# barry-mir/mixing-style-transfer

Hardware: AMD Instinct MI355X
Metric: triplets/sec (10 s @ 44.1 kHz, 4-stem, bs=24) (higher is better)
Workload: dtype f32

## Files before the change

### mixing-style-transfer_amd/csrc/melfeat.hip

```cpp
#include "common.h"
#include "fft_wave.h"
#include "fft_pk.h"
#include "stage_a_tables.h"

#include <algorithm>
#include <cmath>
#include <memory>
#include <vector>


namespace {

constexpr int kWaves = 8;
constexpr int kFPW = 2;
constexpr int kTF = kWaves * kFPW;
constexpr int kTileStride = kTF + 1;
constexpr int kThreads = kWaves * 64;
constexpr int nf_of(int n_fft) { return n_fft >= 2048 ? 1 : kFPW; }
constexpr int kNumScalars = 80;

enum : int {
  S_LOGSUM = 0,
  S_LINSUM = 4,
  S_MASK = 8,
// ... 688 lines not shown
          p.logmel[((size_t)clip * 8 * M + row) * p.F + fb + f] = s_tile[f * TS + row];
    }
    for (int e = tid; e < nf * M; e += kThreads) {
      const int f = e / M, m = e - f * M;
      const float* t = s_tile + f * TS + m;
      float S[4];
#pragma unroll
      for (int s = 0; s < 4; ++s)
        S[s] = 0.5f * ((__expf(t[(2 * s) * M]) - 1e-10f) + (__expf(t[(2 * s + 1) * M]) - 1e-10f));
#pragma unroll
      for (int s = 0; s < 4; ++s) {
        float other = -INFINITY;
#pragma unroll
        for (int j = 0; j < 4; ++j)
          if (j != s) other = fmaxf(other, S[j]);
        mask[s] += __frcp_rn(1.0f + __expf(S[s] - other));
      }
    }
    {
      const int b0 = fb * p.hop, b1 = (fb + nf == p.F) ? p.T : min(p.T, (fb + nf) * p.hop);
      for (int i = b0 + tid * 4; i < b1; i += kThreads * 4) {
        float x[8][4];
#pragma unroll
        for (int c = 0; c < 8; ++c) {
          const ST* src = chan(c) + i;
          if (i + 3 < b1) {
            Smp<ST>::ld4(src, x[c]);
          } else {
#pragma unroll
            for (int e = 0; e < 4; ++e) x[c][e] = (i + e < b1) ? Smp<ST>::ld(src + e) : 0.f;
          }
        }
#pragma unroll
        for (int e = 0; e < 4; ++e) {
          const float mL = ((x[0][e] + x[2][e]) + x[4][e]) + x[6][e];
          const float mR = ((x[1][e] + x[3][e]) + x[5][e]) + x[7][e];
          mixsq = fmaf(mL, mL, mixsq);
          mixsq = fmaf(mR, mR, mixsq);
        }
      }
    }
    __syncthreads();
  }

  float* red = reinterpret_cast<float*>(s_scr);
#pragma unroll
  for (int r = 0; r < NB; ++r) red[(wave * NB + r) * 64 + lane] = acc_db[r];
  float* red2 = red + kWaves * NB * 64;
  {
    const float v[13] = {acc_log, acc_lin, sqL, sqR, dsL, dsR, dqL, dqR, cr, mid, side, mixsq, 0.f};
#pragma unroll
    for (int k = 0; k < 12; ++k) {
      const float r = mst::wave_sum(v[k]);
      if (lane == 0) red2[wave * 24 + k] = r;
    }
    const float a = mst::wave_max(pkL), b = mst::wave_max(pkR);
#pragma unroll
    for (int s = 0; s < 4; ++s) {
      const float r = mst::wave_sum(mask[s]);
      if (lane == 0) red2[wave * 24 + 14 + s] = r;
    }
    if (lane == 0) red2[wave * 24 + 12] = a, red2[wave * 24 + 13] = b;
  }
  __syncthreads();
  for (int i = tid; i < 4 * NB * 64; i += kThreads) {
    const int l = i & 63, r = (i >> 6) % NB, s = i / (64 * NB);
    const int band = p.lanebands[r * 64 + l].band;
    if (band >= 0) {
      float v = 0.f;
#pragma unroll
      for (int w = 0; w < WPS; ++w) v += red[((WPS * s + w) * NB + r) * 64 + l];
      part[s * M + band] = v;
    }
  }
  if (tid < 4) {
    const int s = tid;
    float v[14];
#pragma unroll
    for (int k = 0; k < 14; ++k) v[k] = 0.f;
    for (int w = 0; w < WPS; ++w) {
      const float* a = red2 + (WPS * s + w) * 24;
#pragma unroll
      for (int k = 0; k < 12; ++k) v[k] += a[k];
      v[12] = fmaxf(v[12], a[12]), v[13] = fmaxf(v[13], a[13]);
    }
    float* q = part + 4 * M;
    q[S_LOGSUM + s] = v[0];
    q[S_LINSUM + s] = v[1];
    q[S_SQ + 2 * s] = v[2], q[S_SQ + 2 * s + 1] = v[3];
    q[S_DSUM + 2 * s] = v[4], q[S_DSUM + 2 * s + 1] = v[5];
    q[S_DSQ + 2 * s] = v[6], q[S_DSQ + 2 * s + 1] = v[7];
    q[S_CROSS + s] = v[8];
    q[S_MID + s] = v[9];
    q[S_SIDE + s] = v[10];
    q[S_PEAK + 2 * s] = v[12], q[S_PEAK + 2 * s + 1] = v[13];
    float mk = 0.f;
    for (int w = 0; w < kWaves; ++w) mk += red2[w * 24 + 14 + s];
    q[S_MASK + s] = mk;
    q[S_PIVOT + 2 * s] = Smp<ST>::ld(chan(2 * s) + o_piv), q[S_PIVOT + 2 * s + 1] = Smp<ST>::ld(chan(2 * s + 1) + o_piv);
  }
  if (tid == 8) {
    float mx = 0.f;
    for (int w = 0; w < kWaves; ++w) mx += red2[w * 24 + 11];
    part[4 * M + S_MIX] = mx;
    part[4 * M + S_NSAMP] = (float)max(0, o_end - o_begin);
    part[4 * M + S_NFRAME] = (float)max(0, f_end - f_begin);
  }
}

struct FParams {
  const float* partials;
  float* feats;
  int M, F, T, runs_per_clip, pstride, detailed_bins, feat_dim;
};

__device__ __forceinline__ double wave_sum_f64(double v) {
#pragma unroll
  for (int o = 32; o > 0; o >>= 1) v += __shfl_xor(v, o, 64);
  return v;
}

__device__ double pearson_vs_index(const double* y, int n, int lane) {
  double my = 0;
  for (int i = lane; i < n; i += 64) my += y[i];
  my = wave_sum_f64(my) / n;
  const double mx = 0.5 * (n - 1);
  double sxy = 0, sxx = 0, syy = 0;
  for (int i = lane; i < n; i += 64) {
    const double dx = i - mx, dy = y[i] - my;
    sxy += dx * dy, sxx += dx * dx, syy += dy * dy;
  }
  sxy = wave_sum_f64(sxy), sxx = wave_sum_f64(sxx), syy = wave_sum_f64(syy);
  const double std_unbiased = sqrt(syy / (n - 1));
  if (std_unbiased < 1e-6) return 0.0;
  double c = sxy / sqrt(sxx * syy);
  return fmin(1.0, fmax(-1.0, c));
}

struct FinalizeLds {
  static constexpr int a_sc = 0, a_chmean = a_sc + kNumScalars * 8, a_chm2 = a_chmean + 64, a_cross = a_chm2 + 64, a_curve = a_cross + 64;
  static constexpr size_t bytes(int M, int detailed_bins) { return (size_t)4 * M * 8 + a_curve + (size_t)4 * (detailed_bins > 0 ? detailed_bins : 0) * 8; }
};

__global__ __launch_bounds__(256) void melfeat_finalize_kernel(const FParams p) {
  extern __shared__ __attribute__((aligned(16))) unsigned char smem[];
  using L = FinalizeLds;
  double* band = reinterpret_cast<double*>(smem);
  unsigned char* after_band = reinterpret_cast<unsigned char*>(band + 4 * p.M);
  double* sc = reinterpret_cast<double*>(after_band + L::a_sc);
  double* chmean = reinterpret_cast<double*>(after_band + L::a_chmean);
  double* chm2 = reinterpret_cast<double*>(after_band + L::a_chm2);
  double* cross = reinterpret_cast<double*>(after_band + L::a_cross);
  const int tid = threadIdx.x, clip = blockIdx.x, M = p.M;
  const float* base = p.partials + (size_t)clip * p.runs_per_clip * p.pstride;
  const double inv_n_db = 1.0 / (2.0 * p.F);
  const double k_db = 10.0 / log(10.0);
  for (int i = tid; i < 4 * M; i += 256) {
    double s = 0;
#pragma unroll 8
    for (int r = 0; r < p.runs_per_clip; ++r) s += base[(size_t)r * p.pstride + i];
    band[i] = s * inv_n_db * k_db;
  }
  if (tid < kNumScalars) {
    const bool is_max = tid >= S_PEAK && tid < S_PEAK + 8;
    double s = 0;
#pragma unroll 8
    for (int r = 0; r < p.runs_per_clip; ++r) {
      const double v = base[(size_t)r * p.pstride + 4 * M + tid];
      s = is_max ? fmax(s, v) : s + v;
    }
    sc[tid] = s;
  }
  if (tid < 8) {
    double n = 0, mean = 0, m2 = 0;
    for (int r = 0; r < p.runs_per_clip; ++r) {
      const float* q = base + (size_t)r * p.pstride + 4 * M;
      const double nr = q[S_NSAMP];
      if (nr <= 0) continue;
      const double sr = q[S_DSUM + tid], qr = q[S_DSQ + tid];
      const double mr = q[S_PIVOT + tid] + sr / nr, m2r = fmax(0.0, qr - sr * sr / nr);
      const double d = mr - mean, nt = n + nr;
      m2 += m2r + d * d * n * nr / nt;
      mean += d * nr / nt;
      n = nt;
    }
    chmean[tid] = mean, chm2[tid] = m2;
  } else if (tid >= 64 && tid < 68) {
    const int s = tid - 64;
    double n = 0, mL = 0, mR = 0, c = 0;
    for (int r = 0; r < p.runs_per_clip; ++r) {
      const float* q = base + (size_t)r * p.pstride + 4 * M;
      const double nr = q[S_NSAMP];
      if (nr <= 0) continue;
      const double sL = q[S_DSUM + 2 * s], sR = q[S_DSUM + 2 * s + 1];
      const double mLr = q[S_PIVOT + 2 * s] + sL / nr, mRr = q[S_PIVOT + 2 * s + 1] + sR / nr;
      const double cr = q[S_CROSS + s] - sL * sR / nr;
      const double dL = mLr - mL, dR = mRr - mR, nt = n + nr;
      c += cr + dL * dR * n * nr / nt;
      mL += dL * nr / nt, mR += dR * nr / nt;
      n = nt;
    }
    cross[s] = c;
  }
  __syncthreads();

  const int sd = p.detailed_bins > 0 ? p.detailed_bins + 2 : 5;
  const int ps = 10 + sd;
  float* out = p.feats + (size_t)clip * p.feat_dim;
  const int lane = tid & 63;
  auto put_lane = [&](int idx, double v) {
    float f = (float)v;
    f = fminf(fmaxf(f, -100.0f), 100.0f);
    if (v != v) f = 0.0f;
    out[idx] = f;
  };
  auto put = [&](int idx, double v) {
    if (lane == 0) put_lane(idx, v);
  };
  const double n = (double)p.T;
  auto loud = [&](double ms) { return -0.691 + 10.0 * log10(ms + 1e-10); };
  {
    const int s = tid >> 6;
    const int blk = (s == 1) ? 0 : (s == 2) ? ps : (s == 3) ? 2 * ps + 4 : 3 * ps + 4;
    const double msL = sc[S_SQ + 2 * s] / n, msR = sc[S_SQ + 2 * s + 1] / n;
    const double rmsL = sqrt(msL), rmsR = sqrt(msR);
    const double l_stem = loud((sc[S_SQ + 2 * s] + sc[S_SQ + 2 * s + 1]) / (2 * n));
    const double l_mix = loud(sc[S_MIX] / (2 * n));
    put(blk + 0, rmsL);
    put(blk + 1, rmsR);
    put(blk + 2, 20.0 * log10(sc[S_PEAK + 2 * s] / (rmsL + 1e-8)));
    put(blk + 3, 20.0 * log10(sc[S_PEAK + 2 * s + 1] / (rmsR + 1e-8)));
    put(blk + 4, l_stem);
    put(blk + 5, l_stem);
    put(blk + 6, l_stem - l_mix);
    const double* e = band + s * M;
    const double cnt = 2.0 * M * p.F;
    const double flat = exp(sc[S_LOGSUM + s] / cnt) / (sc[S_LINSUM + s] / cnt + 1e-10);
    int o = blk + 7;
    if (p.detailed_bins == 0) {
      const int q = M / 4;
      double lo = 0, mi = 0, hi = 0;
      for (int i = lane; i < q; i += 64) lo += e[i];
      for (int i = q + lane; i < 3 * q; i += 64) mi += e[i];
      for (int i = 3 * q + lane; i < M; i += 64) hi += e[i];
      lo = wave_sum_f64(lo), mi = wave_sum_f64(mi), hi = wave_sum_f64(hi);
      put(o + 0, lo / q);
      put(o + 1, mi / (2 * q));
      put(o + 2, hi / (M - 3 * q));
      put(o + 3, pearson_vs_index(e, M, lane));
      put(o + 4, flat);
    } else {
      const int nb = p.detailed_bins;
      double* curve = reinterpret_cast<double*>(after_band + L::a_curve) + s * nb;
      for (int i = lane; i < nb; i += 64) {
        if (nb >= M) { curve[i] = e[i]; continue; }
        const float scale = nb > 1 ? (float)(M - 1) / (float)(nb - 1) : 0.f;
        const float src = scale * i;
        int i0 = (int)src;
        if (i0 > M - 1) i0 = M - 1;
        const int i1 = i0 + (i0 < M - 1 ? 1 : 0);
        const double lam = src - (float)i0;
        curve[i] = (1.0 - lam) * e[i0] + lam * e[i1];
      }
      __syncthreads();
      for (int i = lane; i < nb; i += 64) put_lane(o + i, curve[i]);
      put(o + nb, pearson_vs_index(curve, nb, lane));
      put(o + nb + 1, flat);
    }
    o = blk + 7 + sd;
    put(o + 0, 20.0 * log10(rmsL / (rmsR + 1e-8)));
    put(o + 1, cross[s] / (sqrt(chm2[2 * s] * chm2[2 * s + 1]) + 1e-8));
    put(o + 2, (sc[S_SIDE + s] / (4 * n)) / (sc[S_MID + s] / (4 * n) + 1e-8));
    put(2 * ps + s, sc[S_MASK + s] / ((double)M * p.F));
  }
}

template <auto Kernel, typename Params>
int launch_stage_a(const Params& kp, int grid, int threads, size_t lds, hipStream_t st) {
  MST_REQUIRE(lds <= kMaxLds, "mst_melfeat_forward: LDS %zu B exceeds 160 KiB", lds);
  const hipError_t e = mst::launch_lds<Kernel>(dim3(grid), dim3(threads), lds, st, kp);
  if (e != hipSuccess) return mst::fail(MST_EHIP, "stage-A kernel launch failed: %s", hipGetErrorString(e));
  return MST_OK;
}

template <int NFFT, int NB, typename ST>
int launch_melfeat(const KParams& kp, int grid, hipStream_t st) {
  return launch_stage_a<melfeat_kernel<NFFT, NB, ST>>(kp, grid, kThreads, GenericLds<NFFT>::bytes(kp.tw_count, kp.tw2_count, kp.nnz, kp.M, kp.tile_bufs), st);
}
template <int NFFT, typename ST, int WPS>
int launch_melfeat_spw(const KParams& kp, int grid, hipStream_t st) {
  return launch_stage_a<melfeat_spw_kernel<NFFT, ST, WPS>>(kp, grid, SpwGeom<WPS>::THREADS, SpwLds<NFFT, WPS>::bytes(kp.tw2_count, kp.nnz, kp.M), st);
}

#include "melfeat_v2.inc"
#include "melfeat_v2_2048.inc"

}

static_assert(sizeof(stage_a::F2) == sizeof(float2), "stage_a_tables.h's pairs are uploaded as float2");

struct mst_plan {
  int sr, n_fft, hop, n_mels, detailed_bins, feat_dim;
  int batches_per_run;
  mst::DevBuf<float> window;
  struct {
    int nb, nnz, tw_count, tw2_count, glen[4], goff[4];
    mst::DevBuf<float2> tw, tw2, post;
    mst::DevBuf<float> melw;
    mst::DevBuf<LaneBand> lanebands;
  } gen;
  struct {
    bool ok = false;
    int wps = 3;
    int nslot = 0, maxcnt = 0, segw_count = 0, glen[kV2Slots] = {0}, goff[kV2Slots] = {0};
    mst::DevBuf<float2> tw2, tw3, tw4, segw;
    mst::DevBuf<int> start, id, bandtab;
  } sw;
};

namespace {

struct StageAEnv {
  int batches_per_run, spw_wps;
  bool v2_wps2, generic, v2_nostd;
  bool old_kernels;
};
StageAEnv read_stage_a_env() {
  auto num = [](const char* name, int dflt) { const char* e = getenv(name); return e ? atoi(e) : dflt; };
  const char* a = getenv("MST_STAGE_A");
  StageAEnv s;
  s.batches_per_run = getenv("MST_MELFEAT_BATCHES") ? std::max(1, num("MST_MELFEAT_BATCHES", 0)) : 0;
  s.spw_wps = num("MST_SPW_WPS", 3);
  s.v2_wps2 = num("MST_V2_WPS", 0) == 2, s.generic = getenv("MST_MELFEAT_GENERIC"), s.v2_nostd = getenv("MST_V2_NOSTD");
  s.old_kernels = s.generic || (a && (!strcmp(a, "spw") || !strcmp(a, "generic")));
  return s;
}

int frames_per_run_of(const mst_plan* p, int F) {
  if (p->batches_per_run > 0) return p->batches_per_run * kTF;
  int fpr = (F + 31) / 32;
  fpr += fpr & 1;
  return std::max(2 * kTF, fpr);
}
int runs_per_clip(const mst_plan* p, int F) {
  const int fpr = frames_per_run_of(p, F);
  return (F + fpr - 1) / fpr;
}
int pstride_of(const mst_plan* p) { return 4 * p->n_mels + kNumScalars; }

int sw_fpw(const mst_plan* p, int F) { return std::max(1, ((F + 31) / 32 + p->sw.wps - 1) / p->sw.wps); }
int sw_runs(const mst_plan* p, int F) {
  const int fpr = p->sw.wps * sw_fpw(p, F);
  return (F + fpr - 1) / fpr;
}

bool v2_table_is_standard(const mst_plan* p) {
  const auto& t = p->sw;
  return p->n_mels == 128 && t.nslot == 3 && t.maxcnt == 1 && t.glen[0] == 14 && t.glen[1] == 3 && !t.glen[2] && !t.goff[0] && t.goff[1] == 14 && t.goff[2] == 17;
}

}

extern "C" {

int mst_plan_create(mst_plan** out, int sample_rate, int n_fft, int hop, int n_mels, const float* window,
                    const float* fb, int detailed_bins) {
  MST_REQUIRE(out && window && fb, "mst_plan_create: NULL argument");
  *out = nullptr;
  MST_REQUIRE(n_fft == 512 || n_fft == 1024 || n_fft == 2048,
              "mst_plan_create: n_fft=%d unsupported (512, 1024, 2048)", n_fft);
  MST_REQUIRE(hop >= 1 && n_mels >= 4 && n_mels <= 256, "mst_plan_create: bad hop=%d / n_mels=%d", hop, n_mels);
  MST_REQUIRE(detailed_bins >= 0 && detailed_bins <= 256 && (detailed_bins == 0 || detailed_bins < n_mels ||
              detailed_bins == n_mels), "mst_plan_create: bad detailed_bins=%d", detailed_bins);
  std::unique_ptr<mst_plan> p(new mst_plan());
  p->sr = sample_rate, p->n_fft = n_fft, p->hop = hop, p->n_mels = n_mels, p->detailed_bins = detailed_bins;
  const int sd = detailed_bins > 0 ? detailed_bins + 2 : 5;
  p->feat_dim = 4 * (10 + sd) + 4;
  const StageAEnv env = read_stage_a_env();
  p->batches_per_run = env.batches_per_run;
  const int n_bins = n_fft / 2 + 1;
  auto& g = p->gen;
  auto& sw = p->sw;
  const bool v2 = n_fft == 1024 && hop == 256, v4 = n_fft == 2048 && hop == 512 && n_mels <= 128;
  sw.wps = (env.v2_wps2 || n_mels > 128 || v4) ? 2 : 3;
  stage_a::PieceTable t;
  if (v2 || v4) t = stage_a::build_pieces(fb, n_bins, n_mels, v2 ? stage_a::v2_piece_opts(n_mels) : stage_a::v4_piece_opts());
  sw.ok = t.ok, sw.nslot = t.nslot, sw.maxcnt = t.maxcnt, sw.segw_count = (int)t.segw.size();
  for (int r = 0; r < kV2Slots; ++r) sw.glen[r] = t.glen[r], sw.goff[r] = t.goff[r];
  const std::vector<int> bands = !t.ok ? std::vector<int>() : v2 ? stage_a::pack_bands16(t, n_mels, stage_a::kV2Dump) : stage_a::pack_bands8(t, n_mels);
  std::vector<float2> t2(mstpk::kTw2Rows * 64), t3(mstpk::kTw3Rows * 64);
  mstpk::fill_twiddles_host(t2.data(), t3.data());
  const std::vector<stage_a::F2> t4 = v4 ? stage_a::tw4_twiddles() : std::vector<stage_a::F2>();

  g.nb = n_mels <= 128 ? 2 : 4;
  const stage_a::LaneBandTable lb = stage_a::build_lane_bands(fb, n_bins, n_mels, g.nb);
  g.nnz = lb.nnz;
  for (int r = 0; r < 4; ++r) g.glen[r] = lb.glen[r], g.goff[r] = lb.goff[r];
  const std::vector<stage_a::F2> tw = stage_a::fft_twiddles(n_fft / 2), post = stage_a::post_twiddles(n_fft);
  std::vector<stage_a::F2> tw2;
  if (n_fft <= 1024) tw2 = stage_a::fft_twiddles(n_fft);
  g.tw_count = (int)tw.size(), g.tw2_count = (int)tw2.size();
  if (tw2.empty()) tw2.push_back(stage_a::F2{1.f, 0.f});
  auto f2 = [](const std::vector<stage_a::F2>& v) { return reinterpret_cast<const float2*>(v.data()); };
  int rc;
  if ((t.ok && ((rc = sw.tw2.upload(t2.data(), t2.size())) || (rc = sw.tw3.upload(t3.data(), t3.size())) ||
                (v4 && (rc = sw.tw4.upload(f2(t4), t4.size()))) || (rc = sw.segw.upload(f2(t.segw), t.segw.size())) ||
                (rc = sw.start.upload(t.start.data(), t.start.size())) || (rc = sw.id.upload(t.id.data(), t.id.size())) ||
                (rc = sw.bandtab.upload(bands.data(), bands.size())))) ||
      (rc = p->window.upload(window, (size_t)n_fft)) || (rc = g.tw.upload(f2(tw), tw.size())) || (rc = g.tw2.upload(f2(tw2), tw2.size())) ||
      (rc = g.post.upload(f2(post), post.size())) || (rc = g.melw.upload(lb.melw.data(), lb.melw.size())) ||
      (rc = g.lanebands.upload(lb.lanebands.data(), lb.lanebands.size())))
    return rc;
  *out = p.release();
  return MST_OK;
}

void mst_plan_destroy(mst_plan* p) { delete p; }

int mst_plan_frames(const mst_plan* p, int T) { return p ? 1 + T / p->hop : MST_EINVAL; }
int mst_plan_feature_dim(const mst_plan* p) { return p ? p->feat_dim : MST_EINVAL; }

size_t mst_melfeat_workspace_bytes(const mst_plan* p, int B, int T) {
  if (!p || B <= 0 || T <= 0) return 0;
  const int F = 1 + T / p->hop;
  const int runs = std::max(runs_per_clip(p, F), p->sw.ok ? sw_runs(p, F) : 0);
  return mst::align_up((size_t)B * runs * pstride_of(p) * sizeof(float), 256);
}

}

namespace {

struct LogmelOut {
  int layout = MST_LOGMEL_REF;
  void* lo = nullptr;
  unsigned* absmax = nullptr;
};

bool plan_uses_v2(const mst_plan* p) { return p->sw.ok && !read_stage_a_env().old_kernels; }

template <typename Fn>
int with_sample_type(bool pcm16, Fn fn) { return pcm16 ? fn(short{}) : fn(float{}); }
template <typename Fn>
auto with_n_fft(int n_fft, Fn fn) {
  if (n_fft == 512) return fn(std::integral_constant<int, 512>{});
  if (n_fft == 1024) return fn(std::integral_constant<int, 1024>{});
  return fn(std::integral_constant<int, 2048>{});
}

template <typename Params, typename Launch>
int launch_sliding_window(const mst_plan* p, Params& k, const LogmelOut& lmo, bool pcm16, Launch launch) {
  const auto& sw = p->sw;
  k.out_mode = lmo.layout, k.logmel_lo = lmo.lo, k.absmax = lmo.absmax;
  k.tw2 = sw.tw2.get(), k.tw3 = sw.tw3.get(), k.segw = sw.segw.get();
  k.nslot = sw.nslot, k.segw_count = sw.segw_count, k.maxcnt = sw.maxcnt, k.fpw = sw_fpw(p, k.F);
  for (size_t r = 0; r < std::size(k.glen); ++r) k.glen[r] = sw.glen[r], k.goff[r] = sw.goff[r];
  return with_sample_type(pcm16, launch);
}

int launch_v2_2048(const mst_plan* p, K4Params k, const LogmelOut& lmo, bool pcm16, hipStream_t st) {
  k.tw4 = p->sw.tw4.get(), k.pstart = p->sw.start.get(), k.pid = p->sw.id.get(), k.bandtab = p->sw.bandtab.get();
  return launch_sliding_window(p, k, lmo, pcm16, [&](auto s) { return launch_melfeat_v2_2048<decltype(s)>(k, k.B * k.runs_per_clip, st); });
}

int launch_v2(const mst_plan* p, K2Params k, const LogmelOut& lmo, bool pcm16, bool no_std, hipStream_t st) {
  k.segstart = p->sw.start.get(), k.segid = p->sw.id.get(), k.bandtab = reinterpret_cast<const int2*>(p->sw.bandtab.get());
  const bool stdt = v2_table_is_standard(p) && !no_std;
  return launch_sliding_window(p, k, lmo, pcm16, [&](auto s) {
    using ST = decltype(s);
    const int grid = k.B * k.runs_per_clip;
    if (p->n_mels > 128) return launch_melfeat_v2<ST, 2, 4>(k, grid, st);
    return p->sw.wps == 3 ? launch_melfeat_v2<ST, 3>(k, grid, st, stdt) : launch_melfeat_v2<ST, 2>(k, grid, st);
  });
}

size_t generic_lds_bytes(const mst_plan* p, int tile_bufs) {
  return with_n_fft(p->n_fft, [&](auto N) { return GenericLds<N()>::bytes(p->gen.tw_count, p->gen.tw2_count, p->gen.nnz, p->n_mels, tile_bufs); });
}

int launch_generic_or_spw(const mst_plan* p, KParams kp, bool pcm16, const StageAEnv& env, hipStream_t st) {
  const auto& g = p->gen;
  kp.tw = g.tw.get(), kp.tw2 = g.tw2.get(), kp.post = g.post.get(), kp.melw = g.melw.get(), kp.lanebands = g.lanebands.get();
  kp.hop = p->hop, kp.tw_count = g.tw_count, kp.tw2_count = g.tw2_count, kp.nnz = g.nnz;
  for (int r = 0; r < 4; ++r) kp.glen[r] = g.glen[r], kp.goff[r] = g.goff[r];
  kp.frames_per_run = frames_per_run_of(p, kp.F);
  bool base16 = true;
  for (int i = 0; i < 4; ++i) base16 = base16 && (reinterpret_cast<uintptr_t>(kp.stem[i]) & 15) == 0;
  kp.vec_ok = base16 && (kp.T % 2 == 0) && (p->hop % 2 == 0) && (kp.clip_stride % 2 == 0);
  kp.vec4_ok = base16 && (kp.T % 4 == 0) && (p->hop % 4 == 0) && (kp.clip_stride % 4 == 0);
  kp.tile_bufs = generic_lds_bytes(p, 2) <= kMaxLds ? 2 : 1;
  const int grid = kp.B * kp.runs_per_clip, n_fft = p->n_fft, M = p->n_mels;
  const bool spw_ok = kp.vec_ok && kp.vec4_ok && p->hop * 4 == n_fft && M <= 128 && g.nb == 2 && (n_fft == 512 || n_fft == 1024) && !env.generic;
  const bool spw3 = spw_ok && env.spw_wps == 3 && n_fft == 1024 && SpwLds<1024, 3>::bytes(g.tw2_count, g.nnz, M) <= kMaxLds;
  const bool spw2 = spw_ok && !spw3 &&
                    (n_fft == 1024 ? SpwLds<1024, 2>::bytes(g.tw2_count, g.nnz, M) : SpwLds<512, 2>::bytes(g.tw2_count, g.nnz, M)) <= kMaxLds;
  return with_sample_type(pcm16, [&](auto s) {
    using ST = decltype(s);
    if (spw3) return launch_melfeat_spw<1024, ST, 3>(kp, grid, st);
    if (spw2) return n_fft == 1024 ? launch_melfeat_spw<1024, ST, 2>(kp, grid, st) : launch_melfeat_spw<512, ST, 2>(kp, grid, st);
    return with_n_fft(n_fft, [&](auto N) { return g.nb == 2 ? launch_melfeat<N(), 2, ST>(kp, grid, st) : launch_melfeat<N(), 4, ST>(kp, grid, st); });
  });
}

int melfeat_forward_impl(const mst_plan* p, const void* const stems4[4], bool pcm16, long long clip_stride, int B, int T,
                         float* logmel, float* feats, void* workspace, size_t workspace_bytes, void* stream, const LogmelOut& lmo = LogmelOut()) {
  MST_REQUIRE(p && stems4[0] && stems4[1] && stems4[2] && stems4[3], "mst_melfeat_forward: NULL plan/stems");
  MST_REQUIRE(clip_stride >= 2LL * T, "mst_melfeat_forward_stems: clip_stride %lld < 2*T", clip_stride);
  MST_REQUIRE(B > 0 && T > p->n_fft / 2, "mst_melfeat_forward: need B>0 and T > n_fft/2 (reflect pad); B=%d T=%d", B, T);
  MST_REQUIRE((long long)B * 8 * T < (1LL << 40), "mst_melfeat_forward: input too large");
  const size_t need = mst_melfeat_workspace_bytes(p, B, T);
  if (!workspace || workspace_bytes < need)
    return mst::fail(MST_ENOMEM, "mst_melfeat_forward: workspace %zu B < required %zu B", workspace_bytes, need);
  hipStream_t st = reinterpret_cast<hipStream_t>(stream);
  const int F = 1 + T / p->hop;
  const size_t lds = generic_lds_bytes(p, generic_lds_bytes(p, 2) <= kMaxLds ? 2 : 1);
  MST_REQUIRE(lds <= kMaxLds, "mst_melfeat_forward: LDS %zu B exceeds 160 KiB", lds);
  const StageAEnv env = read_stage_a_env();
  const bool use_sw = p->sw.ok && !env.old_kernels;
  MST_REQUIRE(lmo.layout == MST_LOGMEL_REF || use_sw, "mst_melfeat_forward: channel-minor log-mel needs the sliding-window kernels");
  if (lmo.absmax) {
    MST_REQUIRE(lmo.layout != MST_LOGMEL_REF, "mst_melfeat_forward: absmax comes with the channel-minor layouts only");
    MST_HIP_CHECK(hipMemsetAsync(lmo.absmax, 0, (size_t)B * sizeof(unsigned), st));
  }
  const int runs = use_sw ? sw_runs(p, F) : runs_per_clip(p, F);
  auto common = [&](auto k) {
    for (int i = 0; i < 4; ++i) k.stem[i] = stems4[i];
    k.clip_stride = clip_stride, k.logmel = logmel, k.partials = reinterpret_cast<float*>(workspace), k.window = p->window.get();
    k.B = B, k.T = T, k.F = F, k.M = p->n_mels, k.runs_per_clip = runs, k.pstride = pstride_of(p);
    return k;
  };
  const int rc = !use_sw            ? launch_generic_or_spw(p, common(KParams{}), pcm16, env, st)
                 : p->n_fft == 2048 ? launch_v2_2048(p, common(K4Params{}), lmo, pcm16, st)
                                    : launch_v2(p, common(K2Params{}), lmo, pcm16, env.v2_nostd, st);
  if (rc) return rc;
  if (feats) {
    const FParams fp{reinterpret_cast<const float*>(workspace), feats, p->n_mels, F, T, runs, pstride_of(p), p->detailed_bins, p->feat_dim};
    hipLaunchKernelGGL(melfeat_finalize_kernel, dim3(B), dim3(256), FinalizeLds::bytes(p->n_mels, p->detailed_bins), st, fp);
    const hipError_t e = hipGetLastError();
    if (e != hipSuccess) return mst::fail(MST_EHIP, "melfeat_finalize_kernel launch failed: %s", hipGetErrorString(e));
  }
  return MST_OK;
}

}

extern "C" {

int mst_melfeat_forward(const mst_plan* p, const float* stems, int B, int T, float* logmel, float* feats,
                        void* workspace, size_t workspace_bytes, void* stream) {
  MST_REQUIRE(p && stems, "mst_melfeat_forward: NULL plan/stems");
  const void* four[4] = {stems, stems + 2 * (size_t)T, stems + 4 * (size_t)T, stems + 6 * (size_t)T};
  return melfeat_forward_impl(p, four, false, (long long)8 * T, B, T, logmel, feats, workspace, workspace_bytes, stream);
}

int mst_melfeat_forward_stems(const mst_plan* p, const float* const stems4[4], long long clip_stride, int B, int T,
                              float* logmel, float* feats, void* workspace, size_t workspace_bytes, void* stream) {
  MST_REQUIRE(p && stems4, "mst_melfeat_forward: NULL plan/stems");
  const void* four[4] = {stems4[0], stems4[1], stems4[2], stems4[3]};
  return melfeat_forward_impl(p, four, false, clip_stride, B, T, logmel, feats, workspace, workspace_bytes, stream);
}

int mst_melfeat_forward_pcm16(const mst_plan* p, const int16_t* stems, int B, int T, float* logmel, float* feats,
                              void* workspace, size_t workspace_bytes, void* stream) {
  MST_REQUIRE(p && stems, "mst_melfeat_forward_pcm16: NULL plan/stems");
  const void* four[4] = {stems, stems + 2 * (size_t)T, stems + 4 * (size_t)T, stems + 6 * (size_t)T};
  return melfeat_forward_impl(p, four, true, (long long)8 * T, B, T, logmel, feats, workspace, workspace_bytes, stream);
}

int mst_melfeat_forward_stems_pcm16(const mst_plan* p, const int16_t* const stems4[4], long long clip_stride, int B,
                                    int T, float* logmel, float* feats, void* workspace, size_t workspace_bytes,
                                    void* stream) {
  MST_REQUIRE(p && stems4, "mst_melfeat_forward_pcm16: NULL plan/stems");
  const void* four[4] = {stems4[0], stems4[1], stems4[2], stems4[3]};
  return melfeat_forward_impl(p, four, true, clip_stride, B, T, logmel, feats, workspace, workspace_bytes, stream);
}

int mst_plan_layout_supported(const mst_plan* p, int layout) {
  if (!p) return 0;
  if (layout == MST_LOGMEL_REF) return 1;
  return (layout == MST_LOGMEL_CM32 || layout == MST_LOGMEL_CM16) && plan_uses_v2(p) ? 1 : 0;
}

int mst_melfeat_forward_io(const mst_plan* p, const mst_melfeat_io* io, int B, int T, void* workspace, size_t workspace_bytes,
                           void* stream) {
  MST_REQUIRE(p && io, "mst_melfeat_forward_io: NULL plan/io");
  MST_REQUIRE(io->layout >= MST_LOGMEL_REF && io->layout <= MST_LOGMEL_CM16, "mst_melfeat_forward_io: unknown layout %d", io->layout);
  MST_REQUIRE(mst_plan_layout_supported(p, io->layout),
              "mst_melfeat_forward_io: layout %d is not available for this plan (n_fft %d, hop %d: query mst_plan_layout_supported)",
              io->layout, p->n_fft, p->hop);
  MST_REQUIRE(io->layout == MST_LOGMEL_REF || !io->logmel || (reinterpret_cast<uintptr_t>(io->logmel) & 15) == 0,
              "mst_melfeat_forward_io: channel-minor log-mel must be 16-byte aligned");
  MST_REQUIRE(io->layout != MST_LOGMEL_CM16 || !io->logmel_lo || (reinterpret_cast<uintptr_t>(io->logmel_lo) & 15) == 0,
              "mst_melfeat_forward_io: channel-minor log-mel must be 16-byte aligned");
  const LogmelOut lo{io->layout, io->logmel_lo, io->absmax};
  const void* four[4] = {io->stems4[0], io->stems4[1], io->stems4[2], io->stems4[3]};
  return melfeat_forward_impl(p, four, io->pcm16 != 0, io->clip_stride, B, T, static_cast<float*>(io->logmel), io->feats, workspace,
                              workspace_bytes, stream, lo);
}

}
```

### mixing-style-transfer_amd/csrc/melfeat_v2.inc

```

constexpr int kV2Slots = 6;

struct K2Params {
  const void* stem[4];
  long long clip_stride;
  float* logmel;
  void* logmel_lo;
  unsigned* absmax;
  int out_mode;
  float* partials;
  const float* window;
  const float2* tw2;
  const float2* tw3;
  const float2* segw;
  const int* segstart;
  const int* segid;
  const int2* bandtab;
  int B, T, F, M;
  int nslot, glen[kV2Slots], goff[kV2Slots], segw_count;
  int maxcnt;
  int fpw;
  int runs_per_clip, pstride;
};

namespace v2 {
using namespace mstpk;

constexpr int kP2 = 0;
constexpr int kExN = 288;
constexpr int kExDump = kExN - 1;
constexpr int kExHi = 544;
constexpr int kExLo = kExHi + kExN;
static_assert(kExLo + kExN <= kScr, "exchange areas must fit the FFT scratch");
static_assert(kExDump == stage_a::kV2Dump && kV2Slots == stage_a::kMaxSlots, "the piece table is built for these limits");

__device__ __forceinline__ v2f pair_power4(v2f zk, v2f zm) {
  const v2f s = zk + zm, d = zk - zm;
  const v2f q = s * s;
  v2f r;
  asm("v_pk_fma_f32 %0, %1, %1, %2 op_sel:[1,1,0] op_sel_hi:[0,0,1]" : "=v"(r) : "v"(d), "v"(q));
  return r;
}

__device__ __forceinline__ v2f sel2(unsigned long long m, v2f a, v2f b) {
  float rx, ry;
  const float ax = a.x, ay = a.y, bx = b.x, by = b.y;
  asm("v_cndmask_b32 %0, %1, %2, %3" : "=v"(rx) : "v"(bx), "v"(ax), "s"(m));
  asm("v_cndmask_b32 %0, %1, %2, %3" : "=v"(ry) : "v"(by), "v"(ay), "s"(m));
  return mk(rx, ry);
}

template <typename ST>
__device__ __forceinline__ float ld_at(const ST* base, int idx) {
  const unsigned boff = (unsigned)idx * (unsigned)sizeof(ST);
  return Smp<ST>::lds(reinterpret_cast<const ST*>(reinterpret_cast<const char*>(base) + boff));
}

__device__ __forceinline__ v2f bcast_fma(float w, v2f q, v2f acc) { return __builtin_elementwise_fma(mk(w, w), q, acc); }

typedef float f4u __attribute__((ext_vector_type(4), aligned(4)));

typedef float f32x4v __attribute__((ext_vector_type(4)));
typedef _Float16 h16x2 __attribute__((ext_vector_type(2)));

template <int NBL>
struct CmGeom {
  static constexpr int MB = 64 * NBL, PSTR = 2 * MB + 16, TILE = 4 * PSTR;
};
template <int NBL, int BLK>
__device__ __forceinline__ void block_absmax(const float (&out)[2 * NBL][BLK], int lane, int nv, int M, unsigned* s_amax) {
  float bm = 0.f;
#pragma unroll
  for (int r = 0; r < NBL; ++r)
#pragma unroll
    for (int e = 0; e < BLK; ++e)
      if (e < nv && lane + 64 * r < M) bm = fmaxf(bm, fmaxf(fabsf(out[2 * r][e]), fabsf(out[2 * r + 1][e])));
  bm = mst::wave_max(bm);
  if (lane == 0) atomicMax(s_amax, __float_as_uint(bm));
}
template <int NBL, int BLK, int WPS, int SCR>
__device__ __forceinline__ void cm_stage(const float (&out)[2 * NBL][BLK], v2f* s_scr, int h, int stem, int lane, int nv, int out_mode) {
  using G = CmGeom<NBL>;
  static_assert((BLK / 4) * G::TILE <= 2 * SCR, "the staged frames of a wave must fit its FFT scratch");
#pragma unroll
  for (int e = 0; e < BLK; ++e) {
    if (e < nv) {
      float* tl = reinterpret_cast<float*>(s_scr + ((e & 3) * WPS + h) * SCR) + (e >> 2) * G::TILE + stem * G::PSTR;
#pragma unroll
      for (int r = 0; r < NBL; ++r) {
        const float vL = out[2 * r][e], vR = out[2 * r + 1][e];
        v2f val;
        if (out_mode == 2) {
          const _Float16 hL = (_Float16)vL, hR = (_Float16)vR;
          const h16x2 hi = {hL, hR}, lo = {(_Float16)(vL - (float)hL), (_Float16)(vR - (float)hR)};
          val = mk(__builtin_bit_cast(float, hi), __builtin_bit_cast(float, lo));
        } else {
          val = mk(vL, vR);
        }
        *reinterpret_cast<v2f*>(tl + 2 * (lane + 64 * r)) = val;
      }
    }
  }
}
template <int NBL, int BLK>
__device__ __forceinline__ void cm_store(const v2f* scr, int stem, int lane, int nv, size_t frow0, int M, float* logmel, void* logmel_lo,
                                         int out_mode) {
  using G = CmGeom<NBL>;
#pragma unroll
  for (int q = 0; q < BLK / 4; ++q) {
    const int e = 4 * q + stem;
    if (e < nv) {
      const float* tl = reinterpret_cast<const float*>(scr) + q * G::TILE;
      const size_t frow = frow0 + (size_t)e * M;
      if (out_mode == 1) {
        f32x4v* dst = reinterpret_cast<f32x4v*>(logmel) + frow * 2;
#pragma unroll
        for (int it = 0; it < 2 * NBL; ++it) {
          const int g = 64 * it + lane, b = g >> 1, pp = g & 1;
          const v2f a0 = *reinterpret_cast<const v2f*>(tl + (2 * pp) * G::PSTR + 2 * b);
          const v2f a1 = *reinterpret_cast<const v2f*>(tl + (2 * pp + 1) * G::PSTR + 2 * b);
          if (b < M) dst[g] = f32x4v{a0.x, a0.y, a1.x, a1.y};
        }
      } else {
        f32x4v* dhi = reinterpret_cast<f32x4v*>(logmel) + frow;
        f32x4v* dlo = reinterpret_cast<f32x4v*>(logmel_lo) + frow;
#pragma unroll
        for (int it = 0; it < NBL; ++it) {
          const int b = 64 * it + lane;
          v2f a[4];
#pragma unroll
          for (int j = 0; j < 4; ++j) a[j] = *reinterpret_cast<const v2f*>(tl + j * G::PSTR + 2 * b);
          if (b < M) {
            dhi[b] = f32x4v{a[0].x, a[1].x, a[2].x, a[3].x};
            if (logmel_lo) dlo[b] = f32x4v{a[0].y, a[1].y, a[2].y, a[3].y};
          }
        }
      }
    }
  }
}


}

template <int WPS> struct V2Geom {
  static constexpr int BLK = WPS == 2 ? 8 : 4;
  static constexpr int SB = BLK;
  static constexpr bool WIN_LDS = true;
  static constexpr bool MIX_EARLY = WPS == 2;
};

template <int WPS, int NBL>
struct V2Lds {
  static constexpr int BLK = NBL == 2 ? V2Geom<WPS>::BLK : 4, MB = 64 * NBL, WAVES = 4 * WPS;
  static constexpr int tw2 = 0, tw3 = tw2 + mstpk::kTw2Rows * 64 * 8, segw = tw3 + mstpk::kTw3Rows * 64 * 8;
  static constexpr int a_win = 0, a_exch = a_win + (V2Geom<WPS>::WIN_LDS ? 1024 * 4 : 0);
  static constexpr int a_scr = a_exch + WPS * BLK * 4 * MB * 4, a_amax = a_scr + WAVES * mstpk::kScr * 8;
  static constexpr size_t bytes(int segw_count) { return (size_t)segw + (size_t)segw_count * 8 + a_amax + 16; }
  static_assert(WAVES * NBL * 64 + WAVES * 16 <= 2 * WAVES * mstpk::kScr, "the reduction buffer must fit the FFT scratch");
};

template <typename ST, int WPS, int NBL = 2, bool CM = false, bool STD = false>
__global__ __launch_bounds__(WPS * 256) void melfeat_v2_kernel(const K2Params p) {
#pragma clang fp contract(off)
  using namespace mstpk;
  using namespace v2;
  using L = V2Lds<WPS, NBL>;
  constexpr int kWaves = L::WAVES, kThreads = kWaves * 64, BLK = L::BLK, MB = L::MB;
  constexpr bool kUnrollBlock = STD && BLK == 4;
  constexpr bool WIN_LDS = V2Geom<WPS>::WIN_LDS, MIX_EARLY = V2Geom<WPS>::MIX_EARLY;
  constexpr int SB = BLK;
  constexpr float kLn2 = 0.69314718055994530942f;
  extern __shared__ __attribute__((aligned(16))) unsigned char smem[];
  v2f* s_tw2 = reinterpret_cast<v2f*>(smem + L::tw2);
  v2f* s_tw3 = reinterpret_cast<v2f*>(smem + L::tw3);
  v2f* s_segw = reinterpret_cast<v2f*>(smem + L::segw);
  unsigned char* after_segw = reinterpret_cast<unsigned char*>(s_segw + p.segw_count);
  float* s_win = reinterpret_cast<float*>(after_segw + L::a_win);
  float* s_exch = reinterpret_cast<float*>(after_segw + L::a_exch);
  v2f* s_scr = reinterpret_cast<v2f*>(after_segw + L::a_scr);
  unsigned* s_amax = reinterpret_cast<unsigned*>(after_segw + L::a_amax);
  static_assert(!STD || NBL == 2, "the standard table has 128 bands");
  const int M = STD ? 128 : p.M, T = p.T;
  const int nslot = STD ? 3 : p.nslot, maxcnt = STD ? 1 : p.maxcnt;
  constexpr int kStdLen[3] = {14, 3, 0}, kStdOff[3] = {0, 14, 17};
  constexpr bool cm = CM;

  const int tid = threadIdx.x, lane = tid & 63;
  const int wave = __builtin_amdgcn_readfirstlane(tid >> 6);
  const int work = mst::xcd_remap(blockIdx.x, gridDim.x);
  const int clip = work / p.runs_per_clip, run = work % p.runs_per_clip;
  const int fpr = WPS * p.fpw;
  const int f_begin = run * fpr;
  const int f_end = min(p.F, f_begin + fpr);
  {
    const v2f* g2 = reinterpret_cast<const v2f*>(p.tw2);
    const v2f* g3 = reinterpret_cast<const v2f*>(p.tw3);
    const v2f* gs = reinterpret_cast<const v2f*>(p.segw);
    for (int i = tid; i < kTw2Rows * 64; i += kThreads) s_tw2[i] = g2[i];
    for (int i = tid; i < kTw3Rows * 64; i += kThreads) s_tw3[i] = g3[i];
    for (int i = tid; i < p.segw_count; i += kThreads) s_segw[i] = gs[i];
    if (WIN_LDS)
      for (int i = tid; i < 1024; i += kThreads) s_win[i] = p.window[i];
    if (tid == 0) *s_amax = 0u;
  }
  const int stem = wave / WPS, h = wave % WPS;
  auto chan = [&](int c) {
    return static_cast<const ST*>(p.stem[c >> 1]) + (size_t)clip * p.clip_stride + (size_t)(c & 1) * T;
  };
  const ST* const xL = chan(2 * stem);
  const ST* const xR = chan(2 * stem + 1);
  const int o_begin = f_begin * 256;
  const int o_end = (f_end == p.F) ? T : min(T, f_end * 256);
  const int o_piv = min(o_begin, T - 1);
  const float pvL = Smp<ST>::ld(xL + o_piv), pvR = Smp<ST>::ld(xR + o_piv);
  v2f* scr = s_scr + wave * kScr;
  float* exch = s_exch + h * (BLK * 4 * MB);

  v2f wp[8];
#pragma unroll
  for (int q = 0; q < 8; ++q)
    wp[q] = WIN_LDS ? mk(0.f, 0.f) : mk(p.window[lane + 64 * (2 * q)], p.window[lane + 64 * (2 * q + 1)]);
  constexpr int NSL = NBL == 2 ? 3 : kV2Slots;
  int seg_start[NSL], seg_id[NSL];
#pragma unroll
  for (int r = 0; r < NSL; ++r) {
    seg_start[r] = r < nslot ? p.segstart[r * 64 + lane] : 0;
    seg_id[r] = r < nslot ? p.segid[r * 64 + lane] : kExDump;
  }
  int2 btab[NBL];
#pragma unroll
  for (int r = 0; r < NBL; ++r) btab[r] = p.bandtab[r * 64 + lane];
  const int jb = jb_of(lane);
  const bool l0 = lane == 0;

  float acc_db[NBL], acc_log = 0.f, acc_lin = 0.f, acc_mask = 0.f, mixsq = 0.f;
#pragma unroll
  for (int r = 0; r < NBL; ++r) acc_db[r] = 0.f;
  float sqL = 0.f, sqR = 0.f, pkL = 0.f, pkR = 0.f, dsL = 0.f, dsR = 0.f, dqL = 0.f, dqR = 0.f;
  float cr = 0.f, mid = 0.f, side = 0.f;

  const int f0 = f_begin + h * p.fpw;
  const int nfw = max(0, min(p.fpw, f_end - f0));
  auto ld2 = [&](int pos) {
    const int q = reflect_idx(pos, T);
    return mk(ld_at(xL, q), ld_at(xR, q));
  };
  v2f raw[16];
#pragma unroll
  for (int t = 0; t < 16; ++t) raw[t] = mk(0.f, 0.f);
  if (nfw > 0) {
    const int b0 = f0 * 256 - 512 + lane;
#pragma unroll
    for (int t = 0; t < 16; ++t) raw[t] = ld2(b0 + 64 * t);
  }
  __syncthreads();

  constexpr int kMixLead = 2;
#pragma unroll
  for (int k = 0; k < kMixLead; ++k) {
    const int mp0 = (f0 + k) * 256 + 64 * stem + lane;
    if (k < nfw && mp0 < T) {
      float c8[8];
#pragma unroll
      for (int c = 0; c < 8; ++c) c8[c] = ld_at(chan(c), mp0);
      const float mL = ((c8[0] + c8[2]) + c8[4]) + c8[6];
      const float mR = ((c8[1] + c8[3]) + c8[5]) + c8[7];
      mixsq = fmaf(mL, mL, mixsq);
      mixsq = fmaf(mR, mR, mixsq);
    }
  }

  const int nblk = (p.fpw + BLK - 1) / BLK;
  float out[2 * NBL][SB];
#pragma unroll
  for (int k = 0; k < 2 * NBL; ++k)
#pragma unroll
    for (int e = 0; e < SB; ++e) out[k][e] = 0.f;
  auto store_block = [&](int fb0, int cnt) __attribute__((always_inline)) {
    if (!p.logmel || CM) return;
#pragma unroll
    for (int r = 0; r < NBL; ++r) {
      const int b = lane + 64 * r;
      if (b < M) {
#pragma unroll
        for (int c = 0; c < 2; ++c) {
          float* dst = p.logmel + (((size_t)clip * 8 + 2 * stem + c) * M + b) * p.F + fb0;
          const float* o = out[2 * r + c];
#pragma unroll
          for (int e = 0; e < SB; e += 4) {
            if (e + 4 <= cnt) {
              const f4u v4 = f4u{o[e], o[e + 1], o[e + 2], o[e + 3]};
              *reinterpret_cast<f4u*>(dst + e) = v4;
            } else {
#pragma unroll
              for (int q = 0; q < 3; ++q)
                if (e + q < cnt) dst[e + q] = o[e + q];
            }
          }
        }
      }
    }
  };
#pragma unroll 1
  for (int blk = 0; blk < nblk; ++blk) {
    const int nv = max(0, min(BLK, nfw - blk * BLK));
    if constexpr (kUnrollBlock) {
      static_assert(!kUnrollBlock || (BLK == 4 && SB == 4), "the unrolled block rotates 16 registers in 4 frames");
#define MST_FRAME_STATIC 1
      if (0 < nv) {
#define MST_FRAME_I 0
#include "melfeat_v2_frame.inc"
#undef MST_FRAME_I
      }
      if (1 < nv) {
#define MST_FRAME_I 1
#include "melfeat_v2_frame.inc"
#undef MST_FRAME_I
      }
      if (2 < nv) {
#define MST_FRAME_I 2
#include "melfeat_v2_frame.inc"
#undef MST_FRAME_I
      }
      if (3 < nv) {
#define MST_FRAME_I 3
#include "melfeat_v2_frame.inc"
#undef MST_FRAME_I
      }
#undef MST_FRAME_STATIC
    } else {
#define MST_FRAME_STATIC 0
#define MST_FRAME_I fi
#pragma unroll 1
      for (int fi = 0; fi < nv; ++fi)
#include "melfeat_v2_frame.inc"
#undef MST_FRAME_I
#undef MST_FRAME_STATIC
    }
    {
      const int done = min(nfw, (blk + 1) * BLK);
      if (nv > 0 && (done % SB == 0 || done == nfw)) {
        const int cnt = (done - 1) % SB + 1;
        store_block(f0 + done - cnt, cnt);
      }
    }
    __syncthreads();
#pragma unroll
    for (int r = 0; r < NBL; ++r) {
      const int b = lane + 64 * r;
      if (b < M) {
#pragma unroll 2
        for (int e = 0; e < nv; ++e) {
          float other = -INFINITY, own = 0.f;
#pragma unroll
          for (int j = 0; j < 4; ++j) {
            const float sj = exch[(e * 4 + j) * MB + b];
            other = (j != stem) ? fmaxf(other, sj) : other;
            own = (j == stem) ? sj : own;
          }
          acc_mask += __builtin_amdgcn_rcpf(1.0f + __expf(own - other));
        }
      }
    }
    if (cm && p.absmax) block_absmax<NBL, BLK>(out, lane, nv, M, s_amax);
    if (cm && p.logmel) cm_stage<NBL, BLK, WPS, kScr>(out, s_scr, h, stem, lane, nv, p.out_mode);
    __syncthreads();
    if (cm && p.logmel)
      cm_store<NBL, BLK>(scr, stem, lane, nv, ((size_t)clip * p.F + (f0 + blk * BLK)) * M, M, p.logmel, p.logmel_lo, p.out_mode);
  }
  if (cm) __syncthreads();

  float* red = reinterpret_cast<float*>(s_scr);
#pragma unroll
  for (int r = 0; r < NBL; ++r) red[(wave * NBL + r) * 64 + lane] = acc_db[r];
  float* red2 = red + kWaves * NBL * 64;
  {
    const float v[13] = {acc_log, acc_lin, sqL, sqR, dsL, dsR, dqL, dqR, cr, mid, side, mixsq, acc_mask};
#pragma unroll
    for (int k = 0; k < 13; ++k) {
      const float r = mst::wave_sum(v[k]);
      if (lane == 0) red2[wave * 16 + k] = r;
    }
    const float a = mst::wave_max(pkL), b = mst::wave_max(pkR);
    if (lane == 0) red2[wave * 16 + 13] = a, red2[wave * 16 + 14] = b;
  }
  __syncthreads();
  float* part = p.partials + ((size_t)clip * p.runs_per_clip + run) * p.pstride;
  for (int i = tid; i < 4 * MB; i += kThreads) {
    const int s = i / MB, b = i % MB;
    if (b < M) {
      float v = 0.f;
#pragma unroll
      for (int w = 0; w < WPS; ++w) v += red[((WPS * s + w) * NBL + (b >> 6)) * 64 + (b & 63)];
      part[s * M + b] = v;
    }
  }
  if (tid < 4) {
    const int s = tid;
    float v[13], pk0 = 0.f, pk1 = 0.f;
#pragma unroll
    for (int k = 0; k < 13; ++k) v[k] = 0.f;
    for (int w = 0; w < WPS; ++w) {
      const float* a = red2 + (WPS * s + w) * 16;
#pragma unroll
      for (int k = 0; k < 13; ++k) v[k] += a[k];
      pk0 = fmaxf(pk0, a[13]), pk1 = fmaxf(pk1, a[14]);
    }
    float* q = part + 4 * M;
    q[S_LOGSUM + s] = v[0];
    q[S_LINSUM + s] = v[1];
    q[S_SQ + 2 * s] = v[2], q[S_SQ + 2 * s + 1] = v[3];
    q[S_DSUM + 2 * s] = v[4], q[S_DSUM + 2 * s + 1] = v[5];
    q[S_DSQ + 2 * s] = v[6], q[S_DSQ + 2 * s + 1] = v[7];
    q[S_CROSS + s] = v[8];
    q[S_MID + s] = v[9];
    q[S_SIDE + s] = v[10];
    q[S_MASK + s] = v[12];
    q[S_PEAK + 2 * s] = pk0, q[S_PEAK + 2 * s + 1] = pk1;
    q[S_PIVOT + 2 * s] = Smp<ST>::ld(chan(2 * s) + o_piv), q[S_PIVOT + 2 * s + 1] = Smp<ST>::ld(chan(2 * s + 1) + o_piv);
  }
  if (cm && p.absmax && tid == 0) atomicMax(p.absmax + clip, *s_amax);
  if (tid == 8) {
    float mxs = 0.f;
    for (int w = 0; w < kWaves; ++w) mxs += red2[w * 16 + 11];
    part[4 * M + S_MIX] = mxs;
    part[4 * M + S_NSAMP] = (float)max(0, o_end - o_begin);
    part[4 * M + S_NFRAME] = (float)max(0, f_end - f_begin);
  }
}

template <typename ST, int WPS, int NBL = 2>
int launch_melfeat_v2(const K2Params& kp, int grid, hipStream_t st, bool std_table = false) {
  const size_t lds = V2Lds<WPS, NBL>::bytes(kp.segw_count);
  if constexpr (WPS == 3 && NBL == 2)
    if (std_table && kp.out_mode != 0) return launch_stage_a<melfeat_v2_kernel<ST, WPS, NBL, true, true>>(kp, grid, WPS * 256, lds, st);
  return kp.out_mode != 0 ? launch_stage_a<melfeat_v2_kernel<ST, WPS, NBL, true>>(kp, grid, WPS * 256, lds, st)
                          : launch_stage_a<melfeat_v2_kernel<ST, WPS, NBL, false>>(kp, grid, WPS * 256, lds, st);
}
```

Measured before the change: 2853.

## Make v2 melfeat kernel persistent with prefetch of next work item

Launches the v2 sliding-window kernel with a grid capped at the CU count. Each block loops over work items in a grid-stride fashion and issues the next item's raw sample and pivot loads before the current item's reduction and partial-sum stores. This is meant to amortise per-block setup, such as twiddle table staging into LDS, and to hide global load latency behind the epilogue. It adds register pressure, an extra barrier per item, and a risk of lower occupancy from only one block per CU.

```diff
diff --git a/mixing-style-transfer_amd/csrc/melfeat.hip b/mixing-style-transfer_amd/csrc/melfeat.hip
--- a/mixing-style-transfer_amd/csrc/melfeat.hip
+++ b/mixing-style-transfer_amd/csrc/melfeat.hip
@@ -1014,6 +1014,8 @@
 struct mst_plan {
   int sr, n_fft, hop, n_mels, detailed_bins, feat_dim;
   int batches_per_run;
+  bool persistent = true;
+  int cu_count = 0;
   mst::DevBuf<float> window;
   struct {
     int nb, nnz, tw_count, tw2_count, glen[4], goff[4];
@@ -1090,6 +1092,10 @@
   p->feat_dim = 4 * (10 + sd) + 4;
   const StageAEnv env = read_stage_a_env();
   p->batches_per_run = env.batches_per_run;
+  const char* sched = getenv("MST_STAGE_A_SCHEDULE");
+  MST_REQUIRE(!sched || !strcmp(sched, "persistent") || !strcmp(sched, "per-run"),
+              "mst_plan_create: MST_STAGE_A_SCHEDULE=%s (persistent, per-run)", sched);
+  p->persistent = !sched || !strcmp(sched, "persistent");
   const int n_bins = n_fft / 2 + 1;
   auto& g = p->gen;
   auto& sw = p->sw;
@@ -1123,6 +1129,9 @@
       (rc = g.post.upload(f2(post), post.size())) || (rc = g.melw.upload(lb.melw.data(), lb.melw.size())) ||
       (rc = g.lanebands.upload(lb.lanebands.data(), lb.lanebands.size())))
     return rc;
+  int dev = 0;
+  (void)hipGetDevice(&dev);
+  MST_HIP_CHECK(hipDeviceGetAttribute(&p->cu_count, hipDeviceAttributeMultiprocessorCount, dev));
   *out = p.release();
   return MST_OK;
 }
@@ -1178,9 +1187,10 @@
 int launch_v2(const mst_plan* p, K2Params k, const LogmelOut& lmo, bool pcm16, bool no_std, hipStream_t st) {
   k.segstart = p->sw.start.get(), k.segid = p->sw.id.get(), k.bandtab = reinterpret_cast<const int2*>(p->sw.bandtab.get());
   const bool stdt = v2_table_is_standard(p) && !no_std;
+  k.n_items = k.B * k.runs_per_clip;
   return launch_sliding_window(p, k, lmo, pcm16, [&](auto s) {
     using ST = decltype(s);
-    const int grid = k.B * k.runs_per_clip;
+    const int grid = p->persistent ? std::min(k.n_items, std::max(1, p->cu_count)) : k.n_items;
     if (p->n_mels > 128) return launch_melfeat_v2<ST, 2, 4>(k, grid, st);
     return p->sw.wps == 3 ? launch_melfeat_v2<ST, 3>(k, grid, st, stdt) : launch_melfeat_v2<ST, 2>(k, grid, st);
   });
diff --git a/mixing-style-transfer_amd/csrc/melfeat_v2.inc b/mixing-style-transfer_amd/csrc/melfeat_v2.inc
--- a/mixing-style-transfer_amd/csrc/melfeat_v2.inc
+++ b/mixing-style-transfer_amd/csrc/melfeat_v2.inc
@@ -21,6 +21,7 @@
   int maxcnt;
   int fpw;
   int runs_per_clip, pstride;
+  int n_items;
 };
 
 namespace v2 {
@@ -188,11 +189,7 @@
 
   const int tid = threadIdx.x, lane = tid & 63;
   const int wave = __builtin_amdgcn_readfirstlane(tid >> 6);
-  const int work = mst::xcd_remap(blockIdx.x, gridDim.x);
-  const int clip = work / p.runs_per_clip, run = work % p.runs_per_clip;
   const int fpr = WPS * p.fpw;
-  const int f_begin = run * fpr;
-  const int f_end = min(p.F, f_begin + fpr);
   {
     const v2f* g2 = reinterpret_cast<const v2f*>(p.tw2);
     const v2f* g3 = reinterpret_cast<const v2f*>(p.tw3);
@@ -205,15 +202,22 @@
     if (tid == 0) *s_amax = 0u;
   }
   const int stem = wave / WPS, h = wave % WPS;
+  int item = blockIdx.x;
+  int clip = 0, run = 0, f_begin = 0, f_end = 0, f0 = 0, nfw = 0;
+  const ST *xL = nullptr, *xR = nullptr;
   auto chan = [&](int c) {
     return static_cast<const ST*>(p.stem[c >> 1]) + (size_t)clip * p.clip_stride + (size_t)(c & 1) * T;
   };
-  const ST* const xL = chan(2 * stem);
-  const ST* const xR = chan(2 * stem + 1);
-  const int o_begin = f_begin * 256;
-  const int o_end = (f_end == p.F) ? T : min(T, f_end * 256);
-  const int o_piv = min(o_begin, T - 1);
-  const float pvL = Smp<ST>::ld(xL + o_piv), pvR = Smp<ST>::ld(xR + o_piv);
+  auto place = [&](int it) __attribute__((always_inline)) {
+    const int work = mst::xcd_remap(it, p.n_items);
+    clip = work / p.runs_per_clip, run = work % p.runs_per_clip;
+    f_begin = run * fpr;
+    f_end = min(p.F, f_begin + fpr);
+    f0 = f_begin + h * p.fpw;
+    nfw = max(0, min(p.fpw, f_end - f0));
+    xL = chan(2 * stem), xR = chan(2 * stem + 1);
+  };
+  float pvL = 0.f, pvR = 0.f;
   v2f* scr = s_scr + wave * kScr;
   float* exch = s_exch + h * (BLK * 4 * MB);
 
@@ -240,23 +244,69 @@
   float sqL = 0.f, sqR = 0.f, pkL = 0.f, pkR = 0.f, dsL = 0.f, dsR = 0.f, dqL = 0.f, dqR = 0.f;
   float cr = 0.f, mid = 0.f, side = 0.f;
 
-  const int f0 = f_begin + h * p.fpw;
-  const int nfw = max(0, min(p.fpw, f_end - f0));
   auto ld2 = [&](int pos) {
     const int q = reflect_idx(pos, T);
     return mk(ld_at(xL, q), ld_at(xR, q));
   };
+  constexpr int kMixLead = 2;
   v2f raw[16];
-#pragma unroll
-  for (int t = 0; t < 16; ++t) raw[t] = mk(0.f, 0.f);
-  if (nfw > 0) {
-    const int b0 = f0 * 256 - 512 + lane;
-#pragma unroll
-    for (int t = 0; t < 16; ++t) raw[t] = ld2(b0 + 64 * t);
-  }
+  auto first_loads = [&]() __attribute__((always_inline)) {
+    const int o_piv = min(f_begin * 256, T - 1);
+    pvL = Smp<ST>::ld(xL + o_piv), pvR = Smp<ST>::ld(xR + o_piv);
+#pragma unroll
+    for (int t = 0; t < 16; ++t) raw[t] = mk(0.f, 0.f);
+    if (nfw > 0) {
+      const int b0 = f0 * 256 - 512 + lane;
+#pragma unroll
+      for (int t = 0; t < 16; ++t) raw[t] = ld2(b0 + 64 * t);
+    }
+  };
+  place(item);
+  first_loads();
   __syncthreads();
 
-  constexpr int kMixLead = 2;
+  const int nblk = (p.fpw + BLK - 1) / BLK;
+  float out[2 * NBL][SB];
+#pragma unroll
+  for (int k = 0; k < 2 * NBL; ++k)
+#pragma unroll
+    for (int e = 0; e < SB; ++e) out[k][e] = 0.f;
+  auto store_block = [&](int fb0, int cnt) __attribute__((always_inline)) {
+    if (!p.logmel || CM) return;
+#pragma unroll
+    for (int r = 0; r < NBL; ++r) {
+      const int b = lane + 64 * r;
+      if (b < M) {
+#pragma unroll
+        for (int c = 0; c < 2; ++c) {
+          float* dst = p.logmel + (((size_t)clip * 8 + 2 * stem + c) * M + b) * p.F + fb0;
+          const float* o = out[2 * r + c];
+#pragma unroll
+          for (int e = 0; e < SB; e += 4) {
+            if (e + 4 <= cnt) {
+              const f4u v4 = f4u{o[e], o[e + 1], o[e + 2], o[e + 3]};
+              *reinterpret_cast<f4u*>(dst + e) = v4;
+            } else {
+#pragma unroll
+              for (int q = 0; q < 3; ++q)
+                if (e + q < cnt) dst[e + q] = o[e + q];
+            }
+          }
+        }
+      }
+    }
+  };
+#pragma unroll 1
+  for (;;) {
+#pragma unroll
+  for (int r = 0; r < NBL; ++r) acc_db[r] = 0.f;
+  acc_log = acc_lin = acc_mask = mixsq = 0.f;
+  sqL = sqR = pkL = pkR = dsL = dsR = dqL = dqR = 0.f;
+  cr = mid = side = 0.f;
+#pragma unroll
+  for (int k = 0; k < 2 * NBL; ++k)
+#pragma unroll
+    for (int e = 0; e < SB; ++e) out[k][e] = 0.f;
 #pragma unroll
   for (int k = 0; k < kMixLead; ++k) {
     const int mp0 = (f0 + k) * 256 + 64 * stem + lane;
@@ -270,38 +320,6 @@
       mixsq = fmaf(mR, mR, mixsq);
     }
   }
-
-  const int nblk = (p.fpw + BLK - 1) / BLK;
-  float out[2 * NBL][SB];
-#pragma unroll
-  for (int k = 0; k < 2 * NBL; ++k)
-#pragma unroll
-    for (int e = 0; e < SB; ++e) out[k][e] = 0.f;
-  auto store_block = [&](int fb0, int cnt) __attribute__((always_inline)) {
-    if (!p.logmel || CM) return;
-#pragma unroll
-    for (int r = 0; r < NBL; ++r) {
-      const int b = lane + 64 * r;
-      if (b < M) {
-#pragma unroll
-        for (int c = 0; c < 2; ++c) {
-          float* dst = p.logmel + (((size_t)clip * 8 + 2 * stem + c) * M + b) * p.F + fb0;
-          const float* o = out[2 * r + c];
-#pragma unroll
-          for (int e = 0; e < SB; e += 4) {
-            if (e + 4 <= cnt) {
-              const f4u v4 = f4u{o[e], o[e + 1], o[e + 2], o[e + 3]};
-              *reinterpret_cast<f4u*>(dst + e) = v4;
-            } else {
-#pragma unroll
-              for (int q = 0; q < 3; ++q)
-                if (e + q < cnt) dst[e + q] = o[e + q];
-            }
-          }
-        }
-      }
-    }
-  };
 #pragma unroll 1
   for (int blk = 0; blk < nblk; ++blk) {
     const int nv = max(0, min(BLK, nfw - blk * BLK));
@@ -371,23 +389,43 @@
   }
   if (cm) __syncthreads();
 
+  int tid_t = tid;
+  asm volatile("" : "+v"(tid_t));
+  const int wave_t = wave;
+  const int lane_t = tid_t & 63;
+  float* part = p.partials + ((size_t)clip * p.runs_per_clip + run) * p.pstride;
+  const int done_clip = clip;
+  const int o_begin = f_begin * 256;
+  const int o_end = (f_end == p.F) ? T : min(T, f_end * 256);
+  const float n_samp = (float)max(0, o_end - o_begin), n_frame = (float)max(0, f_end - f_begin);
+  float pivL = 0.f, pivR = 0.f;
+  if (tid_t < 4) {
+    const int o_piv = min(o_begin, T - 1);
+    pivL = Smp<ST>::ld(chan(2 * tid_t) + o_piv), pivR = Smp<ST>::ld(chan(2 * tid_t + 1) + o_piv);
+  }
+  const int next = item + (int)gridDim.x;
+  const bool more_items = next < p.n_items;
+  if (more_items) {
+    place(next);
+    first_loads();
+  }
+
   float* red = reinterpret_cast<float*>(s_scr);
 #pragma unroll
-  for (int r = 0; r < NBL; ++r) red[(wave * NBL + r) * 64 + lane] = acc_db[r];
+  for (int r = 0; r < NBL; ++r) red[(wave_t * NBL + r) * 64 + lane_t] = acc_db[r];
   float* red2 = red + kWaves * NBL * 64;
   {
     const float v[13] = {acc_log, acc_lin, sqL, sqR, dsL, dsR, dqL, dqR, cr, mid, side, mixsq, acc_mask};
 #pragma unroll
     for (int k = 0; k < 13; ++k) {
       const float r = mst::wave_sum(v[k]);
-      if (lane == 0) red2[wave * 16 + k] = r;
+      if (lane_t == 0) red2[wave_t * 16 + k] = r;
     }
     const float a = mst::wave_max(pkL), b = mst::wave_max(pkR);
-    if (lane == 0) red2[wave * 16 + 13] = a, red2[wave * 16 + 14] = b;
+    if (lane_t == 0) red2[wave_t * 16 + 13] = a, red2[wave_t * 16 + 14] = b;
   }
   __syncthreads();
-  float* part = p.partials + ((size_t)clip * p.runs_per_clip + run) * p.pstride;
-  for (int i = tid; i < 4 * MB; i += kThreads) {
+  for (int i = tid_t; i < 4 * MB; i += kThreads) {
     const int s = i / MB, b = i % MB;
     if (b < M) {
       float v = 0.f;
@@ -396,8 +434,8 @@
       part[s * M + b] = v;
     }
   }
-  if (tid < 4) {
-    const int s = tid;
+  if (tid_t < 4) {
+    const int s = tid_t;
     float v[13], pk0 = 0.f, pk1 = 0.f;
 #pragma unroll
     for (int k = 0; k < 13; ++k) v[k] = 0.f;
@@ -418,15 +456,20 @@
     q[S_SIDE + s] = v[10];
     q[S_MASK + s] = v[12];
     q[S_PEAK + 2 * s] = pk0, q[S_PEAK + 2 * s + 1] = pk1;
-    q[S_PIVOT + 2 * s] = Smp<ST>::ld(chan(2 * s) + o_piv), q[S_PIVOT + 2 * s + 1] = Smp<ST>::ld(chan(2 * s + 1) + o_piv);
-  }
-  if (cm && p.absmax && tid == 0) atomicMax(p.absmax + clip, *s_amax);
-  if (tid == 8) {
+    q[S_PIVOT + 2 * s] = pivL, q[S_PIVOT + 2 * s + 1] = pivR;
+  }
+  if (cm && p.absmax && tid_t == 0) atomicMax(p.absmax + done_clip, *s_amax);
+  if (tid_t == 8) {
     float mxs = 0.f;
     for (int w = 0; w < kWaves; ++w) mxs += red2[w * 16 + 11];
     part[4 * M + S_MIX] = mxs;
-    part[4 * M + S_NSAMP] = (float)max(0, o_end - o_begin);
-    part[4 * M + S_NFRAME] = (float)max(0, f_end - f_begin);
+    part[4 * M + S_NSAMP] = n_samp;
+    part[4 * M + S_NFRAME] = n_frame;
+  }
+  if (!more_items) break;
+  item = next;
+  if (tid_t == 0) *s_amax = 0u;
+  __syncthreads();
   }
 }
 
```

Measured after the change: 2850, median of 2. No clear change (-0.1%).
